# ucsdmanorlab/PSSR2

Measured on AMD Instinct MI355X. Metric: HR tiles/sec (512^2 4xSR) train, higher is better.
Workload: dtype bf16

## Files before the change

### include/pssr_mi355.h

```cpp
#ifndef PSSR_MI355_H
#define PSSR_MI355_H

#include <stdint.h>

#ifdef __cplusplus
extern "C" {
#endif

typedef void* pssr_stream_t;

enum { PSSR_F32 = 0, PSSR_BF16 = 1, PSSR_F16 = 2 };

enum {
    PSSR_OK = 0,
    PSSR_ERR_ARG = -1,
    PSSR_ERR_LAUNCH = -2,
    PSSR_ERR_UNSUPPORTED = -3
};

int pssr_abi_version(void);
const char* pssr_last_error(void);

int pssr_pack_conv_weight(const float* w_oihw, void* packed, int cout, int cin, int ks,
                          int ci_begin, int ci_count, int mode, const int32_t* n_perm,
// ... 168 lines not shown
                    float beta2, float eps, float weight_decay, int64_t step, float grad_scale,
                    pssr_stream_t stream);
int pssr_adamw_step_dev(float* p, const float* g, float* m, float* v, int64_t n, int64_t* state,
                        float beta1, float beta2, float eps, float weight_decay, float grad_scale,
                        pssr_stream_t stream);
int pssr_amp_check(const float* g, int64_t n, int32_t* amp, pssr_stream_t stream);
int pssr_adamw_step_amp(float* p, const float* g, float* m, float* v, int64_t n, int64_t* state,
                        float beta1, float beta2, float eps, float weight_decay, float grad_scale,
                        int32_t* amp, float growth, float backoff, int interval, pssr_stream_t stream);

int pssr_bilinear_down_u8(const uint8_t* hr, uint8_t* tmp, uint8_t* lr, int planes, int H, int W,
                          int h, int w, pssr_stream_t stream);
int pssr_u8_to_f32(const uint8_t* in, float* out, int64_t n, pssr_stream_t stream);
int pssr_crappify_gaussian(const float* in, float* out, int tiles, int64_t per_tile, float intensity,
                           float gain, float spread, uint64_t seed, uint64_t tile_offset,
                           const double* noise, int flags, const uint64_t* tile_counter,
                           pssr_stream_t stream);
int pssr_crappify_poisson(const float* in, float* out, int tiles, int64_t per_tile, float intensity,
                          float gain, float spread, uint64_t seed, uint64_t tile_offset, int flags,
                          const uint64_t* tile_counter, pssr_stream_t stream);
int pssr_crappify_poisson_samples(const float* in, const double* samples, float* out, int64_t n, double intensity,
                                  double gain, int flags, pssr_stream_t stream);
int pssr_counter_add(uint64_t* counter, uint64_t inc, pssr_stream_t stream);
int pssr_gaussian_blur(const float* in, float* tmp, float* out, int planes, int h, int w, float sigma,
                       float gain, int flags, pssr_stream_t stream);

int pssr_crappify_saltpepper(const float* in, float* out, int tiles, int64_t per_tile, float amount, float gain, float spread,
                             uint64_t seed, uint64_t tile_offset, int flags, const uint64_t* tile_counter, pssr_stream_t stream);
int pssr_gaussian_blur_tiles(const float* in, float* tmp, float* out, int tiles, int planes_per_tile, int h, int w, float sigma,
                             float spread, float gain, uint64_t seed, uint64_t tile_offset, int flags, const uint64_t* tile_counter,
                             pssr_stream_t stream);
typedef struct pssr_gather_item { const uint8_t* src; int sh, sw, rot, flip_axis; } pssr_gather_item;
int pssr_gen_pair_geometry_u8(const pssr_gather_item* items_dev, int n_items, uint8_t* out, int c, int res, pssr_stream_t stream);
typedef struct pssr_sheet_desc { const uint8_t* base; int frames, h, w, reserved; } pssr_sheet_desc;
typedef struct pssr_window_item { int sheet, frame0, y0, x0, rot, flip_axis; } pssr_window_item;
int pssr_gather_windows_u8(const pssr_sheet_desc* sheets_dev, int n_sheets, const pssr_window_item* items_dev, int n_items,
                           uint8_t* out, int c, int res, pssr_stream_t stream);

typedef struct pssr_collage_panel {
    const void* src; int64_t image_stride; int32_t row_pitch, src_h, src_w, is_f32; const int32_t* yi; const int32_t* xi;
} pssr_collage_panel;
int pssr_collage_rows_u8(const pssr_collage_panel* panels, int n_panels, uint8_t* canvas, int64_t canvas_pitch, int row0, int n_images,
                         int h, int w, pssr_stream_t stream);

int64_t pssr_window_attn_workspace_bytes(int B, int H, int W, int heads, int ws);
int pssr_window_attn_fwd(const void* qkv, const float* bias_table, void* out, float* lse, int B, int H, int W, int C, int heads, int ws,
                         int shift, float scale, int dtype, pssr_stream_t stream);
int pssr_window_attn_bwd(const void* qkv, const float* bias_table, const float* lse, const void* dout, void* dqkv, float* dbias_table,
                         void* workspace, int64_t workspace_bytes, int B, int H, int W, int C, int heads, int ws, int shift, float scale,
                         int dtype, pssr_stream_t stream);


int pssr_input_plain(const float* x_nchw, void* out, int n, int c, int h, int w, int out_cs, float pre_scale, float pre_shift,
                     int dtype, pssr_stream_t stream);
int pssr_im2col_dil(const void* in, int in_cs, int in_co, int c, const float* scale, const float* shift, void* col, int cp,
                    int n, int h, int w, int dil, int dtype, pssr_stream_t stream);
int pssr_col2im_dil(const void* dcol, int cp, void* out, int out_cs, int out_co, int c, int n, int h, int w, int dil,
                    const void* y, int y_cs, int y_co, const float* scale, const float* shift, const float* mean,
                    const float* invstd, double* stats, int dtype, pssr_stream_t stream);
int pssr_channel_stats_nhwc(const void* x, int cs, int co, int c, int64_t npix, double* stats, int dtype, pssr_stream_t stream);
int pssr_sum_relu(const void* const* ins, const int* in_cs, const int* in_co, int n_in, void* out, int out_cs, int out_co,
                  int64_t npix, int c, int relu, int dtype, pssr_stream_t stream);
int pssr_relu_mask(const void* dout, int do_cs, int do_co, const void* out, int o_cs, int o_co, void* dz, int dz_cs, int dz_co,
                   int64_t npix, int c, int dtype, pssr_stream_t stream);
int pssr_affine_relu(const void* x, int cs, int co, const float* scale, const float* shift, void* out, int out_cs, int out_co,
                     int64_t npix, int c, int dtype, pssr_stream_t stream);
// ... 163 lines not shown
```

### pssr2_amd/csrc/crappify.hip

```cpp
#include "common.h"
#include "pil_taps.h"

namespace {

__global__ void resample_h_kernel(const uint8_t* __restrict__ in, uint8_t* __restrict__ out, int planes, int H, int W, int w) {
    const int ox = blockIdx.x * blockDim.x + threadIdx.x;
    if (ox >= w) return;
    Taps t; pil_taps(ox, W, w, t);
    for (long row = blockIdx.y; row < (long)planes * H; row += gridDim.y) {
        const uint8_t* src = in + row * W + t.xmin;
        int acc = 1 << (PRECISION_BITS - 1);
        for (int x = 0; x < t.n; ++x) acc += (int)src[x] * t.k[x];
        out[row * w + ox] = clip8(acc);
    }
}
__global__ void resample_v_kernel(const uint8_t* __restrict__ in, uint8_t* __restrict__ out, int planes, int H, int h, int w) {
    const int oy = blockIdx.y;
    Taps t; pil_taps(oy, H, h, t);
    for (int pl = blockIdx.z; pl < planes; pl += gridDim.z)
        for (int ox = blockIdx.x * blockDim.x + threadIdx.x; ox < w; ox += gridDim.x * blockDim.x) {
            const uint8_t* src = in + ((long)pl * H + t.xmin) * w + ox;
            int acc = 1 << (PRECISION_BITS - 1);
            for (int y = 0; y < t.n; ++y) acc += (int)src[(long)y * w] * t.k[y];
            out[((long)pl * h + oy) * w + ox] = clip8(acc);
// ... 10 lines not shown
        const uint64_t k = seed ^ (stream * 0x9E3779B97F4A7C15ull + 0xD1B54A32D192ED03ull);
        key[0] = (uint32_t)k; key[1] = (uint32_t)(k >> 32);
    }
    __device__ __forceinline__ uint4 operator()(uint64_t counter, uint32_t sub) const {
        uint32_t c0 = (uint32_t)counter, c1 = (uint32_t)(counter >> 32), c2 = sub, c3 = 0x1BD11BDAu;
        uint32_t k0 = key[0], k1 = key[1];
#pragma unroll
        for (int r = 0; r < 10; ++r) {
            const uint64_t p0 = (uint64_t)0xD2511F53u * c0, p1 = (uint64_t)0xCD9E8D57u * c2;
            const uint32_t n0 = (uint32_t)(p1 >> 32) ^ c1 ^ k0, n1 = (uint32_t)p1, n2 = (uint32_t)(p0 >> 32) ^ c3 ^ k1, n3 = (uint32_t)p0;
            c0 = n0; c1 = n1; c2 = n2; c3 = n3;
            k0 += 0x9E3779B9u; k1 += 0xBB67AE85u;
        }
        return make_uint4(c0, c1, c2, c3);
    }
};
__device__ __forceinline__ double u01(uint32_t hi, uint32_t lo) {
    const uint64_t v = (((uint64_t)hi << 32) | lo) >> 11;
    return fmin(((double)v + 0.5) * (1.0 / 9007199254740992.0), 1.0 - 1.0 / 9007199254740992.0);
}
__device__ __forceinline__ double normal_from(const uint4& r) {
    const double u1 = u01(r.x, r.y), u2 = u01(r.z, r.w);
    return sqrt(-2.0 * log(u1)) * cos(6.283185307179586476925 * u2);
}
__device__ __forceinline__ double finish(double v, int flags) {
    if (flags & 2) v = rint(v);
    if (flags & 3) v = v < 0.0 ? 0.0 : (v > 255.0 ? 255.0 : v);
    return v;
}
__device__ __forceinline__ double tile_intensity(const Philox& ph, float intensity, float spread) {
    if (!(spread > 0.f)) return intensity;
    const double v = (double)intensity + (double)spread * normal_from(ph(~0ull, 7u));
    return v > 0.0 ? v : 0.0;
}

__global__ void gaussian_noise_kernel(const float* __restrict__ in, float* __restrict__ out, int tiles, long per_tile, float intensity,
                                      float gain, float spread, uint64_t seed, uint64_t tile_offset, const double* __restrict__ noise, int flags,
                                      const uint64_t* __restrict__ tile_counter) {
    if (tile_counter) tile_offset += tile_counter[0];
    const long total = (long)tiles * per_tile;
    for (long i = blockIdx.x * (long)blockDim.x + threadIdx.x; i < total; i += (long)gridDim.x * blockDim.x) {
        const long tile = i / per_tile, pix = i % per_tile;
        double nz;
        if (noise) nz = noise[i];
        else {
            const Philox ph(seed, tile_offset + tile);
            nz = (double)gain + tile_intensity(ph, intensity, spread) * normal_from(ph((uint64_t)pix, 0u));
        }
        out[i] = (float)finish((double)in[i] + nz, flags);
    }
}

__device__ double poisson_draw(const Philox& ph, uint64_t pix, double lam) {
    if (lam <= 0.0) return 0.0;
    uint32_t sub = 1;
    if (lam < 10.0) {
        const double enlam = exp(-lam);
        double prod = 1.0; long x = 0;
        for (int it = 0; it < 64; ++it) {
            const uint4 r = ph(pix, sub++);
            const double u[2] = {u01(r.x, r.y), u01(r.z, r.w)};
            for (int j = 0; j < 2; ++j) { prod *= u[j]; if (prod > enlam) ++x; else return (double)x; }
        }
        return (double)x;
    }
    const double slam = sqrt(lam), loglam = log(lam);
    const double b = 0.931 + 2.53 * slam, a = -0.059 + 0.02483 * b;
    const double invalpha = 1.1239 + 1.1328 / (b - 3.4), vr = 0.9277 - 3.6224 / (b - 2.0);
    for (int it = 0; it < 256; ++it) {
        const uint4 r = ph(pix, sub++);
        const double U = u01(r.x, r.y) - 0.5, V = u01(r.z, r.w);
        const double us = 0.5 - fabs(U);
        const double k = floor((2.0 * a / us + b) * U + lam + 0.43);
        if (us >= 0.07 && V <= vr) return k;
        if (k < 0.0 || (us < 0.013 && V > us)) continue;
        if (log(V) + log(invalpha) - log(a / (us * us) + b) <= -lam + k * loglam - lgamma(k + 1.0)) return k;
    }
    return floor(lam + 0.5);
}

__global__ void poisson_noise_kernel(const float* __restrict__ in, float* __restrict__ out, int tiles, long per_tile, float intensity,
                                     float gain, float spread, uint64_t seed, uint64_t tile_offset, int flags,
                                     const uint64_t* __restrict__ tile_counter) {
    if (tile_counter) tile_offset += tile_counter[0];
    const long total = (long)tiles * per_tile;
    for (long i = blockIdx.x * (long)blockDim.x + threadIdx.x; i < total; i += (long)gridDim.x * blockDim.x) {
        const long tile = i / per_tile, pix = i % per_tile;
        const Philox ph(seed, tile_offset + tile);
        const double x = (double)in[i];
        const double y = poisson_draw(ph, (uint64_t)pix, x > 0.0 ? x : 0.0);
        const double mixv = tile_intensity(ph, intensity, spread);
        out[i] = (float)finish(x * (1.0 - mixv) + y * mixv + (double)gain, flags);
    }
}

__global__ void poisson_samples_kernel(const float* __restrict__ in, const double* __restrict__ samples, float* __restrict__ out, long n,
                                       double intensity, double gain, int flags) {
    const float keep = (float)(1.0 - intensity);
    for (long i = blockIdx.x * (long)blockDim.x + threadIdx.x; i < n; i += (long)gridDim.x * blockDim.x) {
        const float t1 = __fmul_rn(in[i], keep);
        const double v = __dadd_rn(__dadd_rn((double)t1, __dmul_rn(samples[i], intensity)), gain);
        out[i] = (float)finish(v, flags);
    }
}

__global__ void blur_pass_kernel(const float* __restrict__ in, float* __restrict__ out, int planes, int h, int w, float sigma, int axis,
                                 float gain, int flags) {
    const int r = (int)(4.0f * sigma + 0.5f);
    const long total = (long)planes * h * w;
    for (long i = blockIdx.x * (long)blockDim.x + threadIdx.x; i < total; i += (long)gridDim.x * blockDim.x) {
        const int x = i % w, y = (i / w) % h;
        const long base = i - (long)y * w - x;
        double wsum = 0.0, acc = 0.0;
        for (int t = -r; t <= r; ++t) {
            const double wt = exp(-0.5 / ((double)sigma * sigma) * (double)t * t);
            int yy = y, xx = x;
            if (axis == 0) { yy = y + t; yy = yy < 0 ? 0 : (yy >= h ? h - 1 : yy); }
            else { xx = x + t; xx = xx < 0 ? 0 : (xx >= w ? w - 1 : xx); }
            wsum += wt; acc += wt * (double)in[base + (long)yy * w + xx];
        }
        double v = (double)(float)(acc / wsum);
        if (axis == 1) v = finish((double)(float)v + (double)gain, flags);
        out[i] = (float)v;
    }
}
// ... 15 lines not shown
}

__global__ void blur_pass_tiles_kernel(const float* __restrict__ in, float* __restrict__ out, int tiles, int planes_per_tile, int h, int w,
                                       float intensity, float spread, uint64_t seed, uint64_t tile_offset, int axis, float gain, int flags,
                                       const uint64_t* __restrict__ tile_counter) {
    if (tile_counter) tile_offset += tile_counter[0];
    const long per_tile = (long)planes_per_tile * h * w, total = (long)tiles * per_tile;
    for (long i = blockIdx.x * (long)blockDim.x + threadIdx.x; i < total; i += (long)gridDim.x * blockDim.x) {
        const long tile = i / per_tile;
        const Philox ph(seed, tile_offset + tile);
        const double sigma = tile_intensity(ph, intensity, spread);
        const int x = i % w, y = (i / w) % h;
        const long base = i - (long)y * w - x;
        double v = (double)in[i];
        if (sigma > 0.0) {
            const int r = (int)(4.0 * (double)(float)sigma + 0.5);
            double wsum = 0.0, acc = 0.0;
            for (int t = -r; t <= r; ++t) {
                const double wt = exp(-0.5 / (sigma * sigma) * (double)t * t);
                int yy = y, xx = x;
                if (axis == 0) { yy = y + t; yy = yy < 0 ? 0 : (yy >= h ? h - 1 : yy); }
                else { xx = x + t; xx = xx < 0 ? 0 : (xx >= w ? w - 1 : xx); }
                wsum += wt; acc += wt * (double)in[base + (long)yy * w + xx];
            }
            v = (double)(float)(acc / wsum);
        }
        if (axis == 1) v = finish((double)(float)v + (double)gain, flags);
        out[i] = (float)v;
    }
}

struct GatherItem { const uint8_t* src; int sh, sw, rot, flip_axis; };

__global__ void gen_pair_geometry_kernel(const GatherItem* __restrict__ items, uint8_t* __restrict__ out, int c, int res) {
    const GatherItem it = items[blockIdx.y];
    const long per_tile = (long)c * res * res;
    const int size = it.sh < it.sw ? (it.sh < res ? it.sh : res) : (it.sw < res ? it.sw : res);
    const bool exact = it.sh == res && it.sw == res;
    const int sx = exact ? 0 : (it.sh - size) / 2, sy = exact ? 0 : (it.sw - size) / 2;
    for (long i = blockIdx.x * (long)blockDim.x + threadIdx.x; i < per_tile; i += (long)gridDim.x * blockDim.x) {
        int ox = (int)(i % res), oy = (int)((i / res) % res), oc = (int)(i / ((long)res * res));
        if (it.flip_axis == 0) oc = c - 1 - oc;
        if (it.flip_axis == 1 || it.flip_axis == 3) oy = res - 1 - oy;
        if (it.flip_axis == 2 || it.flip_axis == 3) ox = res - 1 - ox;
        int py = oy, px = ox;
        if (it.rot) { py = ox; px = res - 1 - oy; }
        if (size > 1) {
            const int period = 2 * (size - 1);
            py %= period; px %= period;
            if (py >= size) py = period - py;
            if (px >= size) px = period - px;
        } else { py = 0; px = 0; }
        out[blockIdx.y * per_tile + i] = it.src[((long)oc * it.sh + sx + py) * it.sw + sy + px];
    }
}

}

extern "C" {

int pssr_bilinear_down_u8(const uint8_t* hr, uint8_t* tmp, uint8_t* lr, int planes, int H, int W, int h, int w, pssr_stream_t s) {
    PSSR_CHECK(hr && tmp && lr && planes > 0 && H > 0 && W > 0 && h > 0 && w > 0, PSSR_ERR_ARG, "bilinear_down_u8: bad args");
    PSSR_CHECK(H >= h && W >= w && (double)W / w <= 19.0 && (double)H / h <= 19.0, PSSR_ERR_UNSUPPORTED, "bilinear_down_u8: reduction ratio must be in [1, 19]");
    long rows = (long)planes * H;
    const long row_groups = (rows + 15) / 16;
    hipLaunchKernelGGL(resample_h_kernel, dim3(cdiv(w, 64), (unsigned)(row_groups < 65535 ? row_groups : 65535)), dim3(64), 0, (hipStream_t)s, hr, tmp, planes, H, W, w);
    PSSR_LAUNCH_CHECK();
    hipLaunchKernelGGL(resample_v_kernel, dim3(cdiv(w, 128), h, planes < 1024 ? planes : 1024), dim3(128), 0, (hipStream_t)s, tmp, lr, planes, H, h, w);
    PSSR_LAUNCH_CHECK();
    return PSSR_OK;
}

int pssr_u8_to_f32(const uint8_t* in, float* out, int64_t n, pssr_stream_t s) {
    PSSR_CHECK(in && out && n > 0, PSSR_ERR_ARG, "u8_to_f32: bad args");
    hipLaunchKernelGGL(u8_to_f32_kernel, dim3(grid1d(n, 8192)), dim3(256), 0, (hipStream_t)s, in, out, (long)n);
    PSSR_LAUNCH_CHECK();
    return PSSR_OK;
}

int pssr_crappify_gaussian(const float* in, float* out, int tiles, int64_t per_tile, float intensity, float gain, float spread,
                           uint64_t seed, uint64_t tile_offset, const double* noise, int flags, const uint64_t* tile_counter,
                           pssr_stream_t s) {
    PSSR_CHECK(in && out && tiles > 0 && per_tile > 0 && flags >= 0 && flags <= 3, PSSR_ERR_ARG, "crappify_gaussian: bad args");
    hipLaunchKernelGGL(gaussian_noise_kernel, dim3(grid1d((long)tiles * per_tile, 8192)), dim3(256), 0, (hipStream_t)s, in, out, tiles, (long)per_tile,
                       intensity, gain, spread, seed, tile_offset, noise, flags, tile_counter);
    PSSR_LAUNCH_CHECK();
    return PSSR_OK;
// ... 38 lines not shown
int pssr_crappify_saltpepper(const float* in, float* out, int tiles, int64_t per_tile, float amount, float gain, float spread, uint64_t seed,
                             uint64_t tile_offset, int flags, const uint64_t* tile_counter, pssr_stream_t s) {
    PSSR_CHECK(in && out && tiles > 0 && per_tile > 0 && flags >= 0 && flags <= 3 && amount >= 0.f, PSSR_ERR_ARG, "crappify_saltpepper: bad args");
    hipLaunchKernelGGL(saltpepper_kernel, dim3(grid1d((long)tiles * per_tile, 8192)), dim3(256), 0, (hipStream_t)s, in, out, tiles, (long)per_tile,
                       amount, gain, spread, seed, tile_offset, flags, tile_counter);
    PSSR_LAUNCH_CHECK();
    return PSSR_OK;
}

int pssr_gaussian_blur_tiles(const float* in, float* tmp, float* out, int tiles, int planes_per_tile, int h, int w, float sigma, float spread,
                             float gain, uint64_t seed, uint64_t tile_offset, int flags, const uint64_t* tile_counter, pssr_stream_t s) {
    PSSR_CHECK(in && tmp && out && tiles > 0 && planes_per_tile > 0 && h > 0 && w > 0 && sigma >= 0.f && spread >= 0.f && flags >= 0 && flags <= 3,
               PSSR_ERR_ARG, "gaussian_blur_tiles: bad args");
    const long total = (long)tiles * planes_per_tile * h * w;
    hipLaunchKernelGGL(blur_pass_tiles_kernel, dim3(grid1d(total, 8192)), dim3(256), 0, (hipStream_t)s, in, tmp, tiles, planes_per_tile, h, w, sigma,
                       spread, seed, tile_offset, 0, 0.f, 0, tile_counter);
    PSSR_LAUNCH_CHECK();
    hipLaunchKernelGGL(blur_pass_tiles_kernel, dim3(grid1d(total, 8192)), dim3(256), 0, (hipStream_t)s, tmp, out, tiles, planes_per_tile, h, w, sigma,
                       spread, seed, tile_offset, 1, gain, flags, tile_counter);
    PSSR_LAUNCH_CHECK();
    return PSSR_OK;
}

int pssr_gen_pair_geometry_u8(const pssr_gather_item* items_dev, int n_items, uint8_t* out, int c, int res, pssr_stream_t s) {
    PSSR_CHECK(items_dev && out && n_items > 0 && n_items <= 65535 && c > 0 && res > 0, PSSR_ERR_ARG, "gen_pair_geometry: bad args");
    static_assert(sizeof(pssr_gather_item) == sizeof(GatherItem), "pssr_gather_item layout");
    const long per_tile = (long)c * res * res;
    long gx = (per_tile + 255) / 256; if (gx > 256) gx = 256;
    hipLaunchKernelGGL(gen_pair_geometry_kernel, dim3((unsigned)gx, n_items), dim3(256), 0, (hipStream_t)s, (const GatherItem*)items_dev, out, c, res);
    PSSR_LAUNCH_CHECK();
    return PSSR_OK;
}

}
```

### pssr2_amd/data.py

```python
from __future__ import annotations

import glob
import random
import warnings
from pathlib import Path

import numpy as np
import torch
from torch.utils.data import Dataset

from .crappifiers import Crappifier, Poisson
from .util import _force_list


def _square_crop(image, max_res):
    h, w = image.shape[-2:]
    if [h, w] == [max_res] * 2:
        return image
    size = min(h, w, max_res)
    sx, sy = (h - size) // 2, (w - size) // 2
    return image[:, sx:sx + size, sy:sy + size]


def _pad_image(image, res):
    if image.shape[-1] < res:
        p = res - image.shape[-1]
        return np.stack([np.pad(ch, [[0, p], [0, p]], mode="reflect") for ch in image])
    return image


def _slice_center(image, n_frames):
    center, half = image.shape[-3] // 2, n_frames // 2
    if n_frames % 2 == 0:
        return image[..., center - half:center + half, :, :]
    return image[..., center - half:center + half + 1, :, :]
# ... 672 lines not shown
    def check(self, sheet, frame0, y0, x0, c, res):
        f, h, w = self.sheets[sheet].shape
        if not (0 <= frame0 and frame0 + c <= f and 0 <= y0 and y0 + res <= h and 0 <= x0 and x0 + res <= w):
            raise ValueError(f"window (frames {frame0}:{frame0 + c}, rows {y0}:{y0 + res}, columns {x0}:{x0 + res}) leaves sheet {sheet} "
                             f"of shape {(f, h, w)}")

    def gather(self, items, c, res):
        from . import ops
        return ops.gather_windows_u8(self.table, len(self.sheets), items, c, res)


def _uniform_frames(sheets, who, what="sheets"):
    frames = {int(getattr(s, "shape", s)[0]) for s in sheets}
    if len(frames) != 1:
        raise ValueError(f"{who}: n_frames=-1 needs {what} with the same number of frames (a batch has one depth); found {sorted(frames)}")
    return frames.pop()


class _DeviceItems:
    _keep_tensors, _host_items = True, False

    def _no_transforms(self, transforms):
        if transforms is not None:
            raise NotImplementedError(f"{type(self).__name__} applies no host transforms")

    def _row_indices(self, indices):
        indices, n = [int(i) for i in indices], len(self)
        for i in indices:
            if not 0 <= i < n:
                self._check_idx(i, row=True)
        return indices


class _DeviceSynthesis(_DeviceItems):

    def _set_generator(self, device, seed):
        self.tile_counter = torch.zeros(1, dtype=torch.int64, device=device)
        self.gen = DevicePairGenerator(self.lr_scale, self.crappifier, seed=seed, tile_counter=self.tile_counter)

    def device_batch(self, items):
        from . import ops
        out = self._gather_u8(items)
        if self.is_lr:
            return ops.u8_to_f32(out)
        pair = self.gen(out)
        ops.counter_add(self.tile_counter, items.shape[0])
        hr, lr = _center_frames(pair, self.n_frames)
        return hr.contiguous(), lr.contiguous()

    def __getitem__(self, idx, pp=False):
        out = self.device_batch(self.draw_items([idx], pp))
        return out[0] if self.is_lr else (out[0][0], out[1][0])


class _DevicePairs(_DeviceItems):

    def device_pair_batch(self, tables, u8=False):
        from . import ops
        sides = []
        for side, (table, depth, res) in enumerate(zip(tables, self.depths, (self.hr_res, self.hr_res // self.lr_scale))):
            if table.shape[0]:
                sides.append(self._gather_u8(side, table, depth, res))
            else:
                sides.append(torch.empty(0, depth, res, res, dtype=torch.uint8, device=table.device))
        sides = [s.contiguous() for s in _center_frames(sides, self.n_frames)]
        return tuple(s if u8 or not s.shape[0] else ops.u8_to_f32(s) for s in sides)

    def __getitem__(self, idx, pp=False):
        hr, lr = self.device_pair_batch(self.draw_pair_items([idx], pp))
        return hr[0], lr[0]


class DeviceTileDataset(_DeviceSynthesis, ArrayDataset):

    def __init__(self, images, hr_res=512, lr_scale=4, crappifier=Poisson(), val_split=0.1, rotation=True, split_seed=0,
                 transforms=None, names=None, n_frames=-1, device="cuda", seed=0):
        self._no_transforms(transforms)
        super().__init__(images, hr_res, lr_scale, crappifier, val_split, rotation, split_seed, None, names, n_frames)
        if isinstance(self.images, list):
            self.images = [torch.as_tensor(s).to(device).contiguous() for s in self.images]
        else:
            self.images = torch.as_tensor(self.images).to(device).contiguous()
        shapes = _stack_shapes(self.images)
        self.depth = max(self.n_frames) if self.n_frames is not None else _uniform_frames(shapes, type(self).__name__, "stacks")
        self.device = self.images[0].device if isinstance(self.images, list) else self.images.device
        self._set_generator(self.device, seed)
        if isinstance(self.images, list):
            bases = [s.data_ptr() for s in self.images]
        else:
            bases = [self.images.data_ptr() + f * self.images[0].numel() for f in range(len(self.images))]
        self._where = [(f, k, base + k * self.depth * h * w, h, w)
                       for f, (base, (_, h, w), n) in enumerate(zip(bases, shapes, self.slices)) for k in range(n)]

    def __len__(self):
        return len(self._where)

    def draw_items(self, indices, pp=False):
        return _gather_rows([self._where[i][2:] + (self._draw_rotation(i, pp),) for i in self._row_indices(indices)], self.device)

    def _gather_u8(self, items):
        return _gen_pair_geometry_u8(items, self.depth, self.hr_res // self.lr_scale if self.is_lr else self.hr_res, self.device)


class DevicePairedTileDataset(_DevicePairs, PairedArrayDataset):

    def __init__(self, hr_images, lr_images, hr_res=512, lr_scale=4, n_frames=-1, val_split=1, rotation=True, split_seed=None,
# ... 73 lines not shown
```

### pssr2_amd/fastpath.py

```python
from __future__ import annotations

import os

import torch

from . import distributed as D
from .util import SSIMLoss as _SSIMLoss


_CAPTURE_MODE = "thread_local"


def enabled():
    return os.environ.get("PSSR_GRAPH", "1") != "0"


def supports(model, dataset, device):
    if getattr(model, "sync_bn", False) and D.rank_world()[1] > 1:
        return False
    return (enabled() and getattr(model, "_engine", None) is not None and hasattr(dataset, "device_batch") and hasattr(dataset, "draw_items")
            and torch.device(device).type == "cuda" and getattr(dataset, "extra_hr_files", None) is None)


def supports_host(model, dataset, device):
# ... 67 lines not shown
                self.copy_stream.wait_event(self.free_ev[k])
            for dst, src in zip(self.stage[k], tensors):
                dst.copy_(src, non_blocking=True)
                if src.is_cuda:
                    src.record_stream(self.copy_stream)
            ready = torch.cuda.Event()
            ready.record(self.copy_stream)
        main.wait_event(ready)
        for dst, src in zip(self.static, self.stage[k]):
            dst.copy_(src)
        done = torch.cuda.Event()
        done.record(main)
        self.free_ev[k], self.keep[k] = done, tensors
        return self.static


class _Cursor:

    def __init__(self, dataset, batch, capacity, device):
        self.dataset, self.batch = dataset, batch
        self.table = torch.zeros(max(capacity, batch), 3, dtype=torch.int64, device=device)
        self.cursor = torch.zeros(1, dtype=torch.int64, device=device)
        self.ar = torch.arange(batch, device=device)

    def load(self, order):
        rows = self.dataset.draw_items(order)
        if rows.shape[0] > self.table.shape[0]:
            raise RuntimeError("epoch longer than the captured gather table")
        self.table[:rows.shape[0]].copy_(rows)
        self.cursor.zero_()
        return rows.shape[0]

    def next_rows(self):
        rows = self.table[self.ar + self.cursor]
        self.cursor.add_(self.batch)
        return rows

    def tail_rows(self, start, count):
        return self.table[start:start + count]


class TrainStepper:

    WARM = 2

    def __init__(self, model, dataset, batch_size, loss_fn, optim, clamp, image_range, scaler, capacity, device, host=False):
        from .optim import FusedAdamW
        self.model, self.dataset, self.batch, self.loss_fn, self.optim = model, dataset, batch_size, loss_fn, optim
        self.clamp, self.image_range, self.scaler = clamp, image_range, scaler
        self.engine = model._engine
        self.rank, self.world = D.rank_world()
        self.fused = isinstance(optim, FusedAdamW)
        self.amp_dev = scaler is not None and self.fused and self.world == 1 and os.environ.get("PSSR_AMP_DEVICE", "1") != "0"
        self.in_graph_optim = self.fused and self.world == 1 and (scaler is None or self.amp_dev)
        if self.fused:
            optim.device_state = True
        self.scale_dev = (scaler.to_device(device).scale_dev if self.amp_dev else torch.ones(1, device=device)) if scaler is not None else None
        self.host = host
        self.cur = _Cursor(dataset, batch_size, capacity, device) if not host else None
        self.feed = _HostFeed(device) if host else None
        self.device = torch.device(device)
        self.graph, self.outs, self.eager_done = None, None, 0
        self.eager_only = False
        self._reduced = False
        self.split = self.world > 1 and os.environ.get("PSSR_DDP_SPLIT", os.environ.get("PSSR_OVERLAP", "1")) != "0"
        self.graph2, self.split_at = None, 0
        self.comm_events = [] if os.environ.get("PSSR_COMM_STATS") == "1" else None
        self.engine.last_train_stepper = self

# ... 314 lines not shown
```

### pssr2_amd/ops.py

```python
from __future__ import annotations

import ctypes as C

import torch

from . import _lib as L

TORCH_DTYPE = {L.F32: torch.float32, L.BF16: torch.bfloat16, L.F16: torch.float16}


def dtype_code(dt: torch.dtype) -> int:
    if dt == torch.float32:
        return L.F32
    if dt == torch.bfloat16:
        return L.BF16
    if dt == torch.float16:
        return L.F16
    raise ValueError(f"unsupported compute dtype {dt}; use torch.float32, torch.bfloat16 or torch.float16")


def pad_to(v: int, m: int) -> int:
    return (v + m - 1) // m * m


# ... 307 lines not shown


def crappify_poisson(x, intensity, gain, spread, seed, tile_offset, flags, out=None, tile_counter=None):
    out = torch.empty_like(x) if out is None else out
    tiles = x.shape[0]
    L.check(L.lib().pssr_crappify_poisson(L.ptr(x), L.ptr(out), tiles, C.c_int64(x.numel() // tiles), C.c_float(intensity), C.c_float(gain),
                                          C.c_float(spread), C.c_uint64(seed), C.c_uint64(tile_offset), flags, L.ptr(tile_counter),
                                          L.stream_ptr()), "pssr_crappify_poisson")
    return out


def crappify_poisson_samples(x, samples, intensity, gain, flags, out=None):
    out = torch.empty_like(x) if out is None else out
    if samples.dtype != torch.float64 or samples.numel() != x.numel():
        raise ValueError("samples: float64, one per element of x")
    L.check(L.lib().pssr_crappify_poisson_samples(L.ptr(x), L.ptr(samples.contiguous()), L.ptr(out), C.c_int64(x.numel()), C.c_double(intensity),
                                                  C.c_double(gain), flags, L.stream_ptr()), "pssr_crappify_poisson_samples")
    return out


def gaussian_blur(x, sigma, gain, flags):
    h, w = x.shape[-2:]
    planes = x.numel() // (h * w)
    tmp, out = torch.empty_like(x), torch.empty_like(x)
    L.check(L.lib().pssr_gaussian_blur(L.ptr(x), L.ptr(tmp), L.ptr(out), planes, h, w, C.c_float(sigma), C.c_float(gain), flags,
                                       L.stream_ptr()), "pssr_gaussian_blur")
    return out


def counter_add(counter, inc):
    L.check(L.lib().pssr_counter_add(L.ptr(counter), C.c_uint64(inc), L.stream_ptr()), "pssr_counter_add")


def adamw_step_dev(p, g, m, v, state, beta1, beta2, eps, weight_decay, grad_scale=1.0):
    L.check(L.lib().pssr_adamw_step_dev(L.ptr(p), L.ptr(g), L.ptr(m), L.ptr(v), C.c_int64(p.numel()), L.ptr(state), C.c_float(beta1),
                                        C.c_float(beta2), C.c_float(eps), C.c_float(weight_decay), C.c_float(grad_scale),
                                        L.stream_ptr()), "pssr_adamw_step_dev")


def amp_check(g, amp):
    L.check(L.lib().pssr_amp_check(L.ptr(g), C.c_int64(g.numel()), L.ptr(amp), L.stream_ptr()), "pssr_amp_check")


def adamw_step_amp(p, g, m, v, state, beta1, beta2, eps, weight_decay, amp, growth, backoff, interval, grad_scale=1.0):
    L.check(L.lib().pssr_adamw_step_amp(L.ptr(p), L.ptr(g), L.ptr(m), L.ptr(v), C.c_int64(p.numel()), L.ptr(state), C.c_float(beta1),
                                        C.c_float(beta2), C.c_float(eps), C.c_float(weight_decay), C.c_float(grad_scale), L.ptr(amp),
                                        C.c_float(growth), C.c_float(backoff), int(interval), L.stream_ptr()), "pssr_adamw_step_amp")


def input_patchify(x, xpatch, scale, shift, patch, dtype, pre_scale=1 / 128, pre_shift=-1.0):
    n, c, h, w = x.shape
    L.check(L.lib().pssr_input_patchify(L.ptr(x), L.ptr(xpatch), n, c, h, w, patch, xpatch.shape[-1], C.c_float(pre_scale),
                                        C.c_float(pre_shift), L.ptr(scale), L.ptr(shift), dtype, L.stream_ptr()), "pssr_input_patchify")


def input_norm_bwd2(dxcol_a, dxcol_b, dpatch, patch, x, mean, invstd, stats, dtype, pre_scale=1 / 128, pre_shift=-1.0):
    n, c, h, w = x.shape
    col = dxcol_a if dxcol_a is not None else dxcol_b
    L.check(L.lib().pssr_input_norm_bwd2(L.ptr(dxcol_a), L.ptr(dxcol_b), col.shape[-1] if col is not None else 0, L.ptr(dpatch),
                                         dpatch.shape[-1] if dpatch is not None else 0, patch, L.ptr(x), C.c_float(pre_scale),
                                         C.c_float(pre_shift), L.ptr(mean), L.ptr(invstd), n, c, h, w, L.ptr(stats), dtype,
                                         L.stream_ptr()), "pssr_input_norm_bwd2")


def dwconv7_pack_batch(items):
    for k in range(0, len(items), L.DWPACK_BATCH_MAX):
# ... 671 lines not shown
```

Measured before the change: 2430.

## Fuse HR gather, LR downsample and noise into one per-strip pair kernel

Adds a single kernel that, per output strip, reads the gather table entry from the device cursor, gathers the rotated and flipped u8 HR rows into LDS, and writes the f32 HR tile. From the same LDS rows it runs the separable PIL-style downsample and applies Gaussian or Poisson noise before writing LR. This replaces the chain of gather, u8-to-f32, two resample passes and noise kernels, along with their intermediate global buffers and the table-index launches. The cursor and tile counter then advance in a tiny kernel. The risk is extra LDS use and redundant halo rows per strip, and the noise must stay bit-identical to the existing per-pixel Philox streams.

```diff
diff --git a/include/pssr_mi355.h b/include/pssr_mi355.h
--- a/include/pssr_mi355.h
+++ b/include/pssr_mi355.h
@@ -224,6 +224,10 @@
                              pssr_stream_t stream);
 typedef struct pssr_gather_item { const uint8_t* src; int sh, sw, rot, flip_axis; } pssr_gather_item;
 int pssr_gen_pair_geometry_u8(const pssr_gather_item* items_dev, int n_items, uint8_t* out, int c, int res, pssr_stream_t stream);
+int pssr_gen_pair_fused(const pssr_gather_item* items_dev, int64_t table_rows, const int64_t* cursor, int n, int depth, int res, int lr_res,
+                        int noise_kind, float intensity, float gain, float spread, uint64_t seed, uint64_t tile_offset,
+                        const uint64_t* tile_counter, int flags, float* hr, float* lr, pssr_stream_t stream);
+int pssr_pair_advance(int64_t* cursor, uint64_t* tile_counter, int64_t rows, uint64_t tiles, pssr_stream_t stream);
 typedef struct pssr_sheet_desc { const uint8_t* base; int frames, h, w, reserved; } pssr_sheet_desc;
 typedef struct pssr_window_item { int sheet, frame0, y0, x0, rot, flip_axis; } pssr_window_item;
 int pssr_gather_windows_u8(const pssr_sheet_desc* sheets_dev, int n_sheets, const pssr_window_item* items_dev, int n_items,
diff --git a/pssr2_amd/csrc/crappify.hip b/pssr2_amd/csrc/crappify.hip
--- a/pssr2_amd/csrc/crappify.hip
+++ b/pssr2_amd/csrc/crappify.hip
@@ -66,6 +66,10 @@
     if (!(spread > 0.f)) return intensity;
     const double v = (double)intensity + (double)spread * normal_from(ph(~0ull, 7u));
     return v > 0.0 ? v : 0.0;
+}
+
+__device__ __forceinline__ double gaussian_noise_at(const Philox& ph, uint64_t pix, double sigma, float gain) {
+    return (double)gain + sigma * normal_from(ph(pix, 0u));
 }
 
 __global__ void gaussian_noise_kernel(const float* __restrict__ in, float* __restrict__ out, int tiles, long per_tile, float intensity,
@@ -79,7 +83,7 @@
         if (noise) nz = noise[i];
         else {
             const Philox ph(seed, tile_offset + tile);
-            nz = (double)gain + tile_intensity(ph, intensity, spread) * normal_from(ph((uint64_t)pix, 0u));
+            nz = gaussian_noise_at(ph, (uint64_t)pix, tile_intensity(ph, intensity, spread), gain);
         }
         out[i] = (float)finish((double)in[i] + nz, flags);
     }
@@ -113,6 +117,12 @@
     return floor(lam + 0.5);
 }
 
+__device__ __forceinline__ double poisson_mix_at(const Philox& ph, uint64_t pix, double x, float intensity, float spread, float gain) {
+    const double y = poisson_draw(ph, pix, x > 0.0 ? x : 0.0);
+    const double mixv = tile_intensity(ph, intensity, spread);
+    return x * (1.0 - mixv) + y * mixv + (double)gain;
+}
+
 __global__ void poisson_noise_kernel(const float* __restrict__ in, float* __restrict__ out, int tiles, long per_tile, float intensity,
                                      float gain, float spread, uint64_t seed, uint64_t tile_offset, int flags,
                                      const uint64_t* __restrict__ tile_counter) {
@@ -121,10 +131,7 @@
     for (long i = blockIdx.x * (long)blockDim.x + threadIdx.x; i < total; i += (long)gridDim.x * blockDim.x) {
         const long tile = i / per_tile, pix = i % per_tile;
         const Philox ph(seed, tile_offset + tile);
-        const double x = (double)in[i];
-        const double y = poisson_draw(ph, (uint64_t)pix, x > 0.0 ? x : 0.0);
-        const double mixv = tile_intensity(ph, intensity, spread);
-        out[i] = (float)finish(x * (1.0 - mixv) + y * mixv + (double)gain, flags);
+        out[i] = (float)finish(poisson_mix_at(ph, (uint64_t)pix, (double)in[i], intensity, spread, gain), flags);
     }
 }
 
@@ -206,27 +213,190 @@
 
 struct GatherItem { const uint8_t* src; int sh, sw, rot, flip_axis; };
 
+struct GatherGeom { int size, sx, sy; };
+__device__ __forceinline__ GatherGeom gather_geom(const GatherItem& it, int res) {
+    const int size = it.sh < it.sw ? (it.sh < res ? it.sh : res) : (it.sw < res ? it.sw : res);
+    const bool exact = it.sh == res && it.sw == res;
+    return {size, exact ? 0 : (it.sh - size) / 2, exact ? 0 : (it.sw - size) / 2};
+}
+__device__ __forceinline__ int gather_plane(const GatherItem& it, int c, int oc) { return it.flip_axis == 0 ? c - 1 - oc : oc; }
+__device__ __forceinline__ void gather_src(const GatherItem& it, const GatherGeom& g, int res, int oy, int ox, int& row, int& col) {
+    if (it.flip_axis == 1 || it.flip_axis == 3) oy = res - 1 - oy;
+    if (it.flip_axis == 2 || it.flip_axis == 3) ox = res - 1 - ox;
+    int py = oy, px = ox;
+    if (it.rot) { py = ox; px = res - 1 - oy; }
+    if (g.size > 1) {
+        const int period = 2 * (g.size - 1);
+        py %= period; px %= period;
+        if (py >= g.size) py = period - py;
+        if (px >= g.size) px = period - px;
+    } else { py = 0; px = 0; }
+    row = g.sx + py; col = g.sy + px;
+}
+
 __global__ void gen_pair_geometry_kernel(const GatherItem* __restrict__ items, uint8_t* __restrict__ out, int c, int res) {
     const GatherItem it = items[blockIdx.y];
     const long per_tile = (long)c * res * res;
-    const int size = it.sh < it.sw ? (it.sh < res ? it.sh : res) : (it.sw < res ? it.sw : res);
-    const bool exact = it.sh == res && it.sw == res;
-    const int sx = exact ? 0 : (it.sh - size) / 2, sy = exact ? 0 : (it.sw - size) / 2;
+    const GatherGeom g = gather_geom(it, res);
     for (long i = blockIdx.x * (long)blockDim.x + threadIdx.x; i < per_tile; i += (long)gridDim.x * blockDim.x) {
-        int ox = (int)(i % res), oy = (int)((i / res) % res), oc = (int)(i / ((long)res * res));
-        if (it.flip_axis == 0) oc = c - 1 - oc;
-        if (it.flip_axis == 1 || it.flip_axis == 3) oy = res - 1 - oy;
-        if (it.flip_axis == 2 || it.flip_axis == 3) ox = res - 1 - ox;
-        int py = oy, px = ox;
-        if (it.rot) { py = ox; px = res - 1 - oy; }
-        if (size > 1) {
-            const int period = 2 * (size - 1);
-            py %= period; px %= period;
-            if (py >= size) py = period - py;
-            if (px >= size) px = period - px;
-        } else { py = 0; px = 0; }
-        out[blockIdx.y * per_tile + i] = it.src[((long)oc * it.sh + sx + py) * it.sw + sy + px];
-    }
+        const int ox = (int)(i % res), oy = (int)((i / res) % res), oc = (int)(i / ((long)res * res));
+        int row, col;
+        gather_src(it, g, res, oy, ox, row, col);
+        out[blockIdx.y * per_tile + i] = it.src[((long)gather_plane(it, c, oc) * it.sh + row) * it.sw + col];
+    }
+}
+
+constexpr int PAIR_STRIP = 8, PAIR_THREADS = 512, PAIR_LDS_BYTES = 64 * 1024;
+constexpr int PAIR_BATCH = 32, PAIR_BATCH16 = 4;
+enum { PAIR_NOISE_NONE = 0, PAIR_NOISE_GAUSSIAN = 1, PAIR_NOISE_POISSON = 2 };
+
+struct PairShape { int n, depth, res, lr_res, strips, rows_max, kpad, pitch, hpitch; };
+struct PairNoise { int flags; float intensity, gain, spread; uint64_t seed, tile_offset; };
+
+struct PairLds { int stage, himg, total; };
+__host__ __device__ inline PairLds pair_lds(const PairShape& p) {
+    PairLds l;
+    l.stage = (2 + p.kpad) * p.lr_res * 4;
+    l.himg = l.stage + p.rows_max * p.pitch;
+    const int maps = (p.res + p.rows_max) * 4, img = (p.rows_max + 4) * p.hpitch;
+    l.total = l.himg + (maps > img ? maps : img);
+    return l;
+}
+
+struct Walk {
+    int r, c, dr, dc, cols;
+    __device__ __forceinline__ Walk(int start, int step, int cols_) : r(start / cols_), c(start % cols_), dr(step / cols_), dc(step % cols_), cols(cols_) {}
+    __device__ __forceinline__ void next() { r += dr; c += dc; if (c >= cols) { c -= cols; ++r; } }
+};
+
+template <int KIND>
+__global__ __launch_bounds__(PAIR_THREADS) void gen_pair_fused_kernel(const GatherItem* __restrict__ items, long table_rows,
+                                                                      const int64_t* __restrict__ cursor, float* __restrict__ hr,
+                                                                      float* __restrict__ lr, PairShape p, PairNoise nz,
+                                                                      const uint64_t* __restrict__ tile_counter) {
+    extern __shared__ __align__(16) uint8_t pair_smem[];
+    const PairLds L = pair_lds(p);
+    int* const tmin = (int*)pair_smem;
+    int* const tn = tmin + p.lr_res;
+    int* const tk = tn + p.lr_res;
+    uint8_t* const stage = pair_smem + L.stage;
+    uint8_t* const himg = pair_smem + L.himg;
+    int* const ctab = (int*)(pair_smem + L.himg);
+    int* const rtab = ctab + p.res;
+    const int tid = threadIdx.x, wave = tid >> 6, lane = tid & 63;
+    const int id = xcd_remap(blockIdx.x, gridDim.x);
+    const int strip = id % p.strips, plane = (id / p.strips) % p.depth, b = id / (p.strips * p.depth);
+    const int oy0 = strip * PAIR_STRIP, oy1 = oy0 + PAIR_STRIP < p.lr_res ? oy0 + PAIR_STRIP : p.lr_res;
+
+    for (int c = tid; c < p.lr_res; c += PAIR_THREADS) {
+        Taps t; pil_taps(c, p.res, p.lr_res, t);
+        const int n = t.n < p.kpad ? t.n : p.kpad;
+        tmin[c] = t.xmin; tn[c] = n;
+        for (int x = 0; x < p.kpad; ++x) tk[x * p.lr_res + c] = x < n ? t.k[x] : 0;
+    }
+    __syncthreads();
+    const int own0 = (int)((long)oy0 * p.res / p.lr_res), own1 = oy1 == p.lr_res ? p.res : (int)((long)oy1 * p.res / p.lr_res);
+    int row0 = tmin[oy0], row1 = tmin[oy1 - 1] + tn[oy1 - 1];
+    row0 = row0 < own0 ? row0 : own0; row1 = row1 > own1 ? row1 : own1;
+    if (row1 - row0 > p.rows_max) row1 = row0 + p.rows_max;
+    const int nrows = row1 - row0;
+
+    long item = b;
+    if (cursor) item += cursor[0];
+    const bool inside = item >= 0 && item < table_rows;
+    GatherItem it = {nullptr, 1, 1, 0, -1};
+    if (inside) it = items[item];
+    const GatherGeom g = gather_geom(it, p.res);
+    for (int x = tid; x < p.res + nrows; x += PAIR_THREADS) {
+        int row, col;
+        if (x < p.res) { gather_src(it, g, p.res, 0, x, row, col); ctab[x] = it.rot ? row : col; }
+        else { gather_src(it, g, p.res, row0 + x - p.res, 0, row, col); rtab[x - p.res] = it.rot ? col : row; }
+    }
+    __syncthreads();
+    const uint8_t* const src = it.src + (long)gather_plane(it, p.depth, plane) * it.sh * it.sw;
+    const int cfirst = ctab[0] < ctab[p.res - 1] ? ctab[0] : ctab[p.res - 1];
+    if (!inside) {
+        for (int i = tid; i < nrows * p.pitch; i += PAIR_THREADS) stage[i] = 0;
+    } else if (it.rot) {
+        for (int ox0 = wave * PAIR_BATCH; ox0 < p.res; ox0 += PAIR_THREADS / 64 * PAIR_BATCH)
+            for (int r = lane; r < nrows; r += 64) {
+                const int col = rtab[r];
+                uint8_t v[PAIR_BATCH];
+#pragma unroll
+                for (int k = 0; k < PAIR_BATCH; ++k) v[k] = src[(long)ctab[ox0 + k < p.res ? ox0 + k : p.res - 1] * it.sw + col];
+#pragma unroll
+                for (int k = 0; k < PAIR_BATCH; ++k) if (ox0 + k < p.res) stage[r * p.pitch + ox0 + k] = v[k];
+            }
+    } else if (g.size == p.res && (p.res & 15) == 0 && (it.sw & 15) == 0 && (((uintptr_t)src + cfirst) & 15) == 0) {
+        const bool rev = ctab[0] > ctab[p.res - 1];
+        Walk w(tid, PAIR_THREADS, p.res >> 4);
+        while (w.r < nrows) {
+            Walk wl = w;
+            uint4 v[PAIR_BATCH16];
+#pragma unroll
+            for (int k = 0; k < PAIR_BATCH16; ++k, wl.next())
+                v[k] = wl.r < nrows ? *(const uint4*)(src + (long)rtab[wl.r] * it.sw + cfirst + 16 * wl.c) : make_uint4(0u, 0u, 0u, 0u);
+#pragma unroll
+            for (int k = 0; k < PAIR_BATCH16; ++k, w.next()) {
+                if (w.r >= nrows) continue;
+                uint32_t* d = (uint32_t*)(stage + w.r * p.pitch + (rev ? p.res - 16 - 16 * w.c : 16 * w.c));
+                if (rev) { d[0] = __builtin_bswap32(v[k].w); d[1] = __builtin_bswap32(v[k].z); d[2] = __builtin_bswap32(v[k].y); d[3] = __builtin_bswap32(v[k].x); }
+                else { d[0] = v[k].x; d[1] = v[k].y; d[2] = v[k].z; d[3] = v[k].w; }
+            }
+        }
+    } else {
+        for (int r = wave; r < nrows; r += PAIR_THREADS / 64) {
+            const uint8_t* s = src + (long)rtab[r] * it.sw;
+            for (int ox = lane; ox < p.res; ox += 64) stage[r * p.pitch + ox] = s[ctab[ox]];
+        }
+    }
+    __syncthreads();
+
+    float* const hrp = hr + ((long)b * p.depth + plane) * p.res * p.res;
+    for (Walk w(tid, PAIR_THREADS, p.res >> 2); w.r < own1 - own0; w.next()) {
+        const int y = own0 + w.r;
+        const uint32_t v = *(const uint32_t*)(stage + (y - row0) * p.pitch + 4 * w.c);
+        *(float4*)(hrp + (long)y * p.res + 4 * w.c) = make_float4((float)(v & 255u), (float)((v >> 8) & 255u), (float)((v >> 16) & 255u), (float)(v >> 24));
+    }
+    for (Walk w(tid, PAIR_THREADS, p.lr_res); w.r < nrows; w.next()) {
+        const uint8_t* s = stage + w.r * p.pitch + tmin[w.c];
+        const int n = tn[w.c];
+        int acc = 1 << (PRECISION_BITS - 1);
+        for (int x = 0; x < n; x += 4) {
+            const int* k = tk + x * p.lr_res + w.c;
+            acc += (int)s[x] * k[0] + (int)s[x + 1] * k[p.lr_res] + (int)s[x + 2] * k[2 * p.lr_res] + (int)s[x + 3] * k[3 * p.lr_res];
+        }
+        himg[w.r * p.hpitch + w.c] = clip8(acc);
+    }
+    __syncthreads();
+
+    const uint64_t tile_offset = tile_counter ? nz.tile_offset + tile_counter[0] : nz.tile_offset;
+    const Philox ph(nz.seed, tile_offset + (uint64_t)b);
+    const double sigma = KIND == PAIR_NOISE_GAUSSIAN ? tile_intensity(ph, nz.intensity, nz.spread) : 0.0;
+    float* const lrp = lr + ((long)b * p.depth + plane) * p.lr_res * p.lr_res;
+#pragma unroll 2
+    for (Walk w(tid, PAIR_THREADS, p.lr_res); w.r < oy1 - oy0; w.next()) {
+        const int oy = oy0 + w.r;
+        const uint8_t* s = himg + (tmin[oy] - row0) * p.hpitch + w.c;
+        const int n = tn[oy];
+        int acc = 1 << (PRECISION_BITS - 1);
+        for (int y = 0; y < n; y += 4) {
+            const int* k = tk + y * p.lr_res + oy;
+            acc += (int)s[y * p.hpitch] * k[0] + (int)s[(y + 1) * p.hpitch] * k[p.lr_res] + (int)s[(y + 2) * p.hpitch] * k[2 * p.lr_res]
+                 + (int)s[(y + 3) * p.hpitch] * k[3 * p.lr_res];
+        }
+        const float x = (float)clip8(acc);
+        const uint64_t pix = ((uint64_t)plane * p.lr_res + oy) * p.lr_res + w.c;
+        float v = x;
+        if constexpr (KIND == PAIR_NOISE_GAUSSIAN) v = (float)finish((double)x + gaussian_noise_at(ph, pix, sigma, nz.gain), nz.flags);
+        else if constexpr (KIND == PAIR_NOISE_POISSON) v = (float)finish(poisson_mix_at(ph, pix, (double)x, nz.intensity, nz.spread, nz.gain), nz.flags);
+        lrp[(long)oy * p.lr_res + w.c] = v;
+    }
+}
+
+__global__ void pair_advance_kernel(int64_t* cursor, uint64_t* tile_counter, int64_t rows, uint64_t tiles) {
+    if (cursor) cursor[0] += rows;
+    if (tile_counter) tile_counter[0] += tiles;
 }
 
 }
@@ -331,4 +501,47 @@
     return PSSR_OK;
 }
 
-}
+int pssr_gen_pair_fused(const pssr_gather_item* items_dev, int64_t table_rows, const int64_t* cursor, int n, int depth, int res, int lr_res,
+                        int noise_kind, float intensity, float gain, float spread, uint64_t seed, uint64_t tile_offset,
+                        const uint64_t* tile_counter, int flags, float* hr, float* lr, pssr_stream_t s) {
+    PSSR_CHECK(items_dev && hr && lr && table_rows > 0 && n > 0 && depth > 0 && res > 0 && lr_res > 0, PSSR_ERR_ARG, "gen_pair_fused: bad args");
+    PSSR_CHECK(noise_kind >= PAIR_NOISE_NONE && noise_kind <= PAIR_NOISE_POISSON && flags >= 0 && flags <= 3, PSSR_ERR_ARG,
+               "gen_pair_fused: noise kind must be 0 (none), 1 (gaussian) or 2 (poisson), flags in [0, 3]");
+    PSSR_CHECK(cursor || n <= table_rows, PSSR_ERR_ARG, "gen_pair_fused: %d items from a table of %lld rows", n, (long long)table_rows);
+    PSSR_CHECK(((uintptr_t)items_dev & 7) == 0 && ((uintptr_t)lr & 3) == 0, PSSR_ERR_ARG, "gen_pair_fused: misaligned table or lr");
+    const double scale = (double)res / lr_res;
+    PSSR_CHECK(res >= lr_res && scale <= 19.0, PSSR_ERR_UNSUPPORTED, "gen_pair_fused: reduction ratio must be in [1, 19]");
+    PSSR_CHECK((res & 3) == 0 && ((uintptr_t)hr & 15) == 0, PSSR_ERR_UNSUPPORTED, "gen_pair_fused: hr rows are written 16 bytes at a time (res %% 4, alignment)");
+    PairShape p;
+    p.n = n; p.depth = depth; p.res = res; p.lr_res = lr_res;
+    p.strips = cdiv(lr_res, PAIR_STRIP);
+    const int kmax = (int)ceil(2.0 * scale) + 2, rows = (int)ceil((PAIR_STRIP + 1) * scale) + 2;
+    p.kpad = ((kmax < 40 ? kmax : 40) + 3) & ~3;
+    p.rows_max = rows < res ? rows : res;
+    p.pitch = res + 4;
+    if ((p.pitch >> 2) % 2 == 0) p.pitch += 4;
+    p.hpitch = lr_res;
+    const PairLds L = pair_lds(p);
+    PSSR_CHECK(L.total <= PAIR_LDS_BYTES, PSSR_ERR_UNSUPPORTED, "gen_pair_fused: res %d -> %d needs %d bytes of LDS per strip (budget %d)", res, lr_res,
+               L.total, PAIR_LDS_BYTES);
+    const long per_tile = (long)depth * res * res, blocks = (long)n * depth * p.strips;
+    PSSR_CHECK(per_tile < (1l << 31) && blocks < (1l << 31), PSSR_ERR_UNSUPPORTED, "gen_pair_fused: tile or grid beyond the 32-bit index range");
+    static_assert(sizeof(pssr_gather_item) == sizeof(GatherItem), "pssr_gather_item layout");
+    PairNoise nz;
+    nz.flags = flags; nz.intensity = intensity; nz.gain = gain; nz.spread = spread; nz.seed = seed; nz.tile_offset = tile_offset;
+    const auto kernel = noise_kind == PAIR_NOISE_GAUSSIAN ? gen_pair_fused_kernel<PAIR_NOISE_GAUSSIAN>
+                      : noise_kind == PAIR_NOISE_POISSON ? gen_pair_fused_kernel<PAIR_NOISE_POISSON> : gen_pair_fused_kernel<PAIR_NOISE_NONE>;
+    hipLaunchKernelGGL(kernel, dim3((unsigned)blocks), dim3(PAIR_THREADS), (size_t)L.total, (hipStream_t)s, (const GatherItem*)items_dev,
+                       (long)table_rows, cursor, hr, lr, p, nz, tile_counter);
+    PSSR_LAUNCH_CHECK();
+    return PSSR_OK;
+}
+
+int pssr_pair_advance(int64_t* cursor, uint64_t* tile_counter, int64_t rows, uint64_t tiles, pssr_stream_t s) {
+    PSSR_CHECK(cursor || tile_counter, PSSR_ERR_ARG, "pair_advance: no counter");
+    hipLaunchKernelGGL(pair_advance_kernel, dim3(1), dim3(1), 0, (hipStream_t)s, cursor, tile_counter, rows, tiles);
+    PSSR_LAUNCH_CHECK();
+    return PSSR_OK;
+}
+
+}
diff --git a/pssr2_amd/data.py b/pssr2_amd/data.py
--- a/pssr2_amd/data.py
+++ b/pssr2_amd/data.py
@@ -1,6 +1,7 @@
 from __future__ import annotations
 
 import glob
+import os
 import random
 import warnings
 from pathlib import Path
@@ -739,14 +740,57 @@
         return indices
 
 
+_PAIR_FUSE = os.environ.get("PSSR_PAIR_FUSE", "1") != "0"
+
+
+class TableRows:
+
+    def __init__(self, table, cursor, ar):
+        self.table, self.cursor, self.ar = table, cursor, ar
+        self.shape = (ar.shape[0], 3)
+
+    def take(self):
+        rows = self.table[self.ar + self.cursor]
+        self.cursor.add_(self.ar.shape[0])
+        return rows
+
+
 class _DeviceSynthesis(_DeviceItems):
+    _gather_rows_fusable = False
 
     def _set_generator(self, device, seed):
         self.tile_counter = torch.zeros(1, dtype=torch.int64, device=device)
         self.gen = DevicePairGenerator(self.lr_scale, self.crappifier, seed=seed, tile_counter=self.tile_counter)
 
+    def fused_pair_stage(self):
+        if not (_PAIR_FUSE and self._gather_rows_fusable) or self.is_lr or not (self.n_frames is None or self.n_frames[0] == self.n_frames[1]):
+            return None
+        spec = self.crappifier.device_spec() if self.crappifier is not None else None
+        if spec is None or (isinstance(spec, tuple) and spec[0] in ("gaussian", "poisson")):
+            return (spec,)
+        return None
+
+    def _fused_batch(self, items):
+        from . import ops
+        stage = self.fused_pair_stage()
+        if stage is None:
+            return None
+        through = isinstance(items, TableRows)
+        n = items.shape[0]
+        pair = ops.gen_pair_fused(items.table if through else items.contiguous(), n, self.depth, self.hr_res, self.hr_res // self.lr_scale,
+                                  stage[0], self.gen.seed, 0, ops.ROUND_CLIP if stage[0] is not None else 0,
+                                  cursor=items.cursor if through else None, tile_counter=self.tile_counter)
+        if pair is not None:
+            ops.pair_advance(items.cursor if through else None, self.tile_counter, n, n)
+        return pair
+
     def device_batch(self, items):
         from . import ops
+        pair = self._fused_batch(items)
+        if pair is not None:
+            return pair
+        if isinstance(items, TableRows):
+            items = items.take()
         out = self._gather_u8(items)
         if self.is_lr:
             return ops.u8_to_f32(out)
@@ -779,6 +823,7 @@
 
 
 class DeviceTileDataset(_DeviceSynthesis, ArrayDataset):
+    _gather_rows_fusable = True
 
     def __init__(self, images, hr_res=512, lr_scale=4, crappifier=Poisson(), val_split=0.1, rotation=True, split_seed=0,
                  transforms=None, names=None, n_frames=-1, device="cuda", seed=0):
diff --git a/pssr2_amd/fastpath.py b/pssr2_amd/fastpath.py
--- a/pssr2_amd/fastpath.py
+++ b/pssr2_amd/fastpath.py
@@ -123,9 +123,10 @@
         return rows.shape[0]
 
     def next_rows(self):
-        rows = self.table[self.ar + self.cursor]
-        self.cursor.add_(self.batch)
-        return rows
+        from .data import TableRows
+        rows = TableRows(self.table, self.cursor, self.ar)
+        fused = getattr(self.dataset, "fused_pair_stage", None)
+        return rows if fused is not None and fused() is not None else rows.take()
 
     def tail_rows(self, start, count):
         return self.table[start:start + count]
diff --git a/pssr2_amd/ops.py b/pssr2_amd/ops.py
--- a/pssr2_amd/ops.py
+++ b/pssr2_amd/ops.py
@@ -363,6 +363,29 @@
     L.check(L.lib().pssr_counter_add(L.ptr(counter), C.c_uint64(inc), L.stream_ptr()), "pssr_counter_add")
 
 
+PAIR_NOISE = {None: 0, "gaussian": 1, "poisson": 2}
+UNSUPPORTED = -3
+
+
+def gen_pair_fused(table, n, depth, res, lr_res, stage=None, seed=0, tile_offset=0, flags=0, cursor=None, tile_counter=None):
+    kind, intensity, gain, spread = stage if stage is not None else (None, 0.0, 0.0, 0.0)
+    if table.dtype != torch.int64 or not table.is_cuda or not table.is_contiguous() or table.dim() != 2 or table.shape[1] != 3:
+        raise ValueError("gen_pair_fused needs a contiguous int64 [rows, 3] gather table on the device")
+    hr = torch.empty(n, depth, res, res, dtype=torch.float32, device=table.device)
+    lr = torch.empty(n, depth, lr_res, lr_res, dtype=torch.float32, device=table.device)
+    status = L.lib().pssr_gen_pair_fused(L.ptr(table), C.c_int64(table.shape[0]), L.ptr(cursor), n, depth, res, lr_res, PAIR_NOISE[kind],
+                                         C.c_float(intensity), C.c_float(gain), C.c_float(spread), C.c_uint64(seed), C.c_uint64(tile_offset),
+                                         L.ptr(tile_counter), flags, L.ptr(hr), L.ptr(lr), L.stream_ptr())
+    if status == UNSUPPORTED:
+        return None
+    L.check(status, "pssr_gen_pair_fused")
+    return hr, lr
+
+
+def pair_advance(cursor, tile_counter, rows, tiles):
+    L.check(L.lib().pssr_pair_advance(L.ptr(cursor), L.ptr(tile_counter), C.c_int64(rows), C.c_uint64(tiles), L.stream_ptr()), "pssr_pair_advance")
+
+
 def adamw_step_dev(p, g, m, v, state, beta1, beta2, eps, weight_decay, grad_scale=1.0):
     L.check(L.lib().pssr_adamw_step_dev(L.ptr(p), L.ptr(g), L.ptr(m), L.ptr(v), C.c_int64(p.numel()), L.ptr(state), C.c_float(beta1),
                                         C.c_float(beta2), C.c_float(eps), C.c_float(weight_decay), C.c_float(grad_scale),
```

New measurement: 2453 (median of 4 runs). No clear change (+0.9%).
